# zakuro-ai/asr

Measured on AMD Instinct MI355X. Metric: utterances/sec (10 s, 161-bin) DS2 5x1024 BiGRU CTC train step, higher is better.
Workload: dtype bf16

## Files before the change

asr_amd/_lib.py:

```python
from __future__ import annotations

import ctypes as C
import os
from typing import Optional

_HERE = os.path.dirname(os.path.abspath(__file__))
LIB_PATH = os.environ.get("DS2_LIB_PATH") or os.path.join(_HERE, "lib", "libds2hip.so")

_lib: Optional[C.CDLL] = None

vp, i32, i64, f32, f64, sz = C.c_void_p, C.c_int, C.c_longlong, C.c_float, C.c_double, C.c_size_t

SIGNATURES = {
    "ds2_version": (C.c_char_p, []),
    "ds2_last_error": (C.c_char_p, []),
    "ds2_device_info": (i32, [C.POINTER(i32), C.POINTER(i32), C.c_char_p, i32]),
    "ds2_debug_flags": (i32, [vp, i32]),
    "ds2_rnn_ctx_init": (i32, [vp, vp, vp, vp]),
    "ds2_memset_async": (i32, [vp, i32, sz, vp]),
    "ds2_ablation_build": (i32, []),
    "ds2_rnn_persistent_status": (i32, [vp, vp]),
    "ds2_rnn_persistent_counters": (i32, [vp, vp]),
    "ds2_rnn_poison_if_starved": (i32, [vp, vp, sz, vp]),
    "ds2_rnn_poison_seen": (i32, [vp]),
# ... 21 lines not shown
    "ds2_cast_f32_from_bf16": (i32, [vp, vp, i64, vp]),
    "ds2_rnn_fwd_x": (i32, [vp, i32, vp, vp, vp, vp, vp, vp, vp, i32, i32, i32, vp, vp, vp, vp, sz, vp]),
    "ds2_split_bf16": (i32, [vp, i32, vp, i32, i32, i32, i32, vp]),
    "ds2_cast_transpose_bf16": (i32, [vp, i32, vp, i32, i32, i32, vp]),
    "ds2_cast_bf16_both_workspace_bytes": (sz, [i32, i32]),
    "ds2_cast_bf16_both": (i32, [vp, i32, vp, i32, vp, i32, i32, i32, vp, vp, sz, vp]),
    "ds2_transpose_bf16": (i32, [vp, i32, vp, i32, i32, i32, vp, vp, sz, vp]),
    "ds2_colreduce_workspace_bytes": (sz, [i32, i32]),
    "ds2_colstats_f32": (i32, [vp, i32, i32, i32, vp, vp, vp, vp, f32, vp, sz, vp]),
    "ds2_add_colstats_f32": (i32, [vp, i32, vp, i32, vp, i32, i32, i32, vp, vp, vp, vp, f32, vp, sz, vp]),
    "ds2_colsum_f32": (i32, [vp, i32, i32, i32, vp, vp, vp, sz, vp]),
    "ds2_bn1d_apply_f32": (i32, [vp, i32, vp, i32, i32, i32, vp, vp, vp, vp, f32, vp]),
    "ds2_bn1d_apply_bf16": (i32, [vp, i32, vp, i32, i32, i32, vp, vp, vp, vp, f32, vp]),
    "ds2_bn1d_bwd_f32": (i32, [vp, i32, vp, i32, vp, i32, i32, i32, vp, vp, vp, f32, vp, vp, vp, sz, vp]),
    "ds2_bn1d_bwd_xbf16": (i32, [vp, i32, vp, i32, vp, i32, i32, i32, vp, vp, vp, f32, vp, vp, vp, sz, vp]),
    "ds2_center_colstats": (i32, [vp, i32, vp, i32, vp, i32, vp, i32, i32, i32, vp, vp, vp, vp, vp, f32, vp, sz, vp]),
    "ds2_wih_fold_bf16": (i32, [vp, i32, vp, i32, i32, vp, vp, vp, vp, f32, vp, i32, vp, vp, vp, vp]),
    "ds2_scale_rank1_f32": (i32, [vp, i32, i32, i32, vp, vp, vp, vp]),
    "ds2_chanreduce_workspace_bytes": (sz, [i32]),
    "ds2_bn2d_stats_f32": (i32, [vp, i32, i32, i32, i32, vp, vp, vp, vp, f32, vp, sz, vp]),
    "ds2_bn2d_act_fwd_f32": (i32, [vp, vp, i32, i32, i32, i32, vp, vp, vp, vp, vp, f32, vp]),
    "ds2_bn2d_act_bwd_f32": (i32, [vp, vp, vp, i32, i32, i32, i32, vp, vp, vp, vp, vp, f32, vp, vp, vp, sz, vp]),
    "ds2_bn2d_act_fwd_fused": (i32, [vp, i32, i32, i32, vp, vp, vp, vp, vp, f32, vp, vp, vp, vp]),
    "ds2_bn2d_act_collapse": (i32, [vp, i32, i32, i32, vp, vp, vp, vp, vp, f32, vp, vp, i32, vp]),
    "ds2_bn2d_act_bwd_fused_workspace_bytes": (sz, [i32, i32, i32]),
    "ds2_bn2d_act_bwd_fused": (i32, [vp, vp, i32, i32, i32, vp, vp, vp, vp, vp, f32, vp, vp, vp, vp, vp, vp, vp, sz, vp]),
    "ds2_transpose_bft_f32": (i32, [vp, vp, i32, i32, i32, i32, vp]),
    "ds2_transpose2d_f32": (i32, [vp, i32, i64, vp, i32, i64, i32, i32, i32, vp]),
    "ds2_conv_dims": (None, [i32, i32, C.POINTER(i32), C.POINTER(i32), C.POINTER(i32)]),
    "ds2_conv_packed_floats": (sz, [i32]),
# ... 122 lines not shown
```

asr_amd/csrc/conv_bf16.hip:

```cpp
#include "common.h"
#include <stdlib.h>

namespace {

typedef __bf16 bf16x8 __attribute__((ext_vector_type(8)));

constexpr int TT = 128, KT = 11, PT = 5, CH = 32;
constexpr int NPIX = TT + KT - 1;
constexpr int IPITCH = 80;
constexpr int WROW = KT * 2 * 2 * 32 * 16;

__device__ __attribute__((aligned(16))) float g_zero_cb[4] = {0.f, 0.f, 0.f, 0.f};

struct CArgs {
  const __bf16* in;
  const __bf16* wpk;
  const float* bias;
  float* out;
  const int* lens;
  int B, Din, T, Dtot, KD, SD, PD, OS, OO;
  int gx, gy, gz;
};

constexpr int IN_CHUNKS = NPIX * 4;
// ... 18 lines not shown
    bx = pair % a.gx; bz = pair / a.gx;
  }
  const int t0 = bx * TT, o0 = R * by, b = bz;
  const int len = a.lens ? min(a.lens[b], a.T) : a.T;
  const int t = t0 + wave * 32 + l31;
  auto out_ptr = [&](int o, int co) { return a.out + (((long long)b * CH + co) * a.Dtot + (a.OS * o + a.OO)) * a.T + t; };
  if (t0 >= len) {
    if (t < a.T) {
#pragma unroll
      for (int q = 0; q < R; ++q)
        if (o0 + q < n_out) {
#pragma unroll
          for (int r = 0; r < 16; ++r) *out_ptr(o0 + q, (r & 3) + 8 * (r >> 2) + 4 * half) = 0.f;
        }
    }
    return;
  }
  f32x16 acc[R];
#pragma unroll
  for (int q = 0; q < R; ++q)
#pragma unroll
    for (int r = 0; r < 16; ++r) acc[q][r] = 0.f;

  const int f0 = SD * o0 - a.PD;
  f32x4 ri[IN_IT], rw[W_IT];
  auto load_in = [&](int f) {
    const bool rowok = f >= 0 && f < a.Din;
    const char* rowp = reinterpret_cast<const char*>(a.in + (((long long)b * a.Din + (rowok ? f : 0)) * a.T) * CH);
#pragma unroll
    for (int u = 0; u < IN_IT; ++u) {
// ... 166 lines not shown
  return 0;
}

extern "C" int ds2_conv2_fwd_bf16_stat_blocks(int B, int D1, int T) {
  const int D2 = (D1 + 2 * 10 - 21) / 2 + 1;
  return ceil_div(T, TT) * ceil_div(D2, 3) * B;
}

extern "C" int ds2_conv2_fwd_bf16_stats(const void* a1_nhwc, const void* wf, const float* bias, const int* lens_dev, float* y2, int B, int D1,
                                        int T, float* stat_part, void* stream) {
  DS2_REQUIRE(a1_nhwc && wf && y2, "ds2_conv2_fwd_bf16: null pointer");
  const int D2 = (D1 + 2 * 10 - 21) / 2 + 1;
  CArgs a{};
  a.in = (const __bf16*)a1_nhwc; a.wpk = (const __bf16*)wf; a.bias = bias; a.out = y2; a.lens = lens_dev;
  a.B = B; a.Din = D1; a.T = T; a.Dtot = D2; a.KD = 21; a.SD = 2; a.PD = 10; a.OS = 1; a.OO = 0;
  if (stat_part) DS2_HIP(hipMemsetAsync(stat_part, 0, (size_t)ds2_conv2_fwd_bf16_stat_blocks(B, D1, T) * 64 * sizeof(float), (hipStream_t)stream));
  a.gx = ceil_div(T, TT); a.gy = ceil_div(D2, 3); a.gz = B;
  hipLaunchKernelGGL((conv2_bf16_rows_kernel<2, 3>), dim3(a.gx * a.gy * a.gz), dim3(256), 0, (hipStream_t)stream, a, D2, stat_part);
  DS2_LAUNCH_CHECK("conv2_bf16_rows_kernel fwd");
  return 0;
}

extern "C" int ds2_conv2_fwd_bf16(const void* a1_nhwc, const void* wf, const float* bias, const int* lens_dev, float* y2, int B, int D1,
                                  int T, void* stream) {
  return ds2_conv2_fwd_bf16_stats(a1_nhwc, wf, bias, lens_dev, y2, B, D1, T, nullptr, stream);
}

extern "C" int ds2_conv2_dgrad_bf16(const void* dy2_nhwc, const void* wd0, const void* wd1, float* da1, int B, int D1, int T, void* stream) {
  DS2_REQUIRE(dy2_nhwc && wd0 && wd1 && da1, "ds2_conv2_dgrad_bf16: null pointer");
  const int D2 = (D1 + 2 * 10 - 21) / 2 + 1;
  for (int p = 0; p < 2; ++p) {
// ... 422 lines not shown
```

asr_amd/csrc/norm.hip:

```cpp
#include "common.h"
#include <algorithm>

namespace {

typedef float f32x4_dw __attribute__((ext_vector_type(4), aligned(4)));
typedef __bf16 nbf16x4 __attribute__((ext_vector_type(4)));
constexpr int BN_ROWS_PER_BLOCK = 32;
__device__ __forceinline__ f32x4 ld4(const float* __restrict__ p, int valid, bool vec) {
  f32x4 v = {0.f, 0.f, 0.f, 0.f};
  if (valid >= 4 && vec) {
    v = *reinterpret_cast<const f32x4*>(p);
  } else if (valid >= 4) {
    const f32x4_dw q = *reinterpret_cast<const f32x4_dw*>(p);
    v.x = q.x; v.y = q.y; v.z = q.z; v.w = q.w;
  } else {
    if (valid > 0) v.x = p[0];
    if (valid > 1) v.y = p[1];
    if (valid > 2) v.z = p[2];
    if (valid > 3) v.w = p[3];
  }
  return v;
}
__device__ __forceinline__ void st4(float* __restrict__ p, f32x4 v, int valid, bool vec) {
  if (valid >= 4 && vec) {
// ... 48 lines not shown
  red[rg][cq * 4 + 0][0] = s0.x; red[rg][cq * 4 + 0][1] = s1.x;
  red[rg][cq * 4 + 1][0] = s0.y; red[rg][cq * 4 + 1][1] = s1.y;
  red[rg][cq * 4 + 2][0] = s0.z; red[rg][cq * 4 + 2][1] = s1.z;
  red[rg][cq * 4 + 3][0] = s0.w; red[rg][cq * 4 + 3][1] = s1.w;
  __syncthreads();
  if (threadIdx.x < 128) {
    const int c = threadIdx.x >> 1, w = threadIdx.x & 1;
    float s = 0.f;
#pragma unroll
    for (int g = 0; g < 16; ++g) s += red[g][c][w];
    const int col = blockIdx.x * 64 + c;
    if (col < H) part[((long long)blockIdx.y * H + col) * 2 + w] = s;
  }
}

__global__ __launch_bounds__(256) void col_finalize_kernel(const float* __restrict__ part, int chunks, int H, double count, int kind,
                                                           float* __restrict__ out0, float* __restrict__ out1,
                                                           float* __restrict__ run_mean, float* __restrict__ run_var, float momentum) {
  __shared__ double red[8][32][2];
  const int cl = threadIdx.x & 31, grp = threadIdx.x >> 5;
  const int c = blockIdx.x * 32 + cl;
  double a = 0.0, b = 0.0;
  if (c < H) {
    double a1 = 0.0, b1 = 0.0, a2 = 0.0, b2 = 0.0, a3 = 0.0, b3 = 0.0;
    int k = grp;
    for (; k + 24 < chunks; k += 32) {
      const float2 p0 = *reinterpret_cast<const float2*>(part + ((long long)k * H + c) * 2);
      const float2 p1 = *reinterpret_cast<const float2*>(part + ((long long)(k + 8) * H + c) * 2);
      const float2 p2 = *reinterpret_cast<const float2*>(part + ((long long)(k + 16) * H + c) * 2);
      const float2 p3 = *reinterpret_cast<const float2*>(part + ((long long)(k + 24) * H + c) * 2);
      a += (double)p0.x; b += (double)p0.y; a1 += (double)p1.x; b1 += (double)p1.y;
      a2 += (double)p2.x; b2 += (double)p2.y; a3 += (double)p3.x; b3 += (double)p3.y;
    }
    for (; k < chunks; k += 8) {
      a += (double)part[((long long)k * H + c) * 2 + 0];
      b += (double)part[((long long)k * H + c) * 2 + 1];
// ... 14 lines not shown
  }
  if (kind == 0) {
    const double m = a / count;
    double v = b / count - m * m;
    if (v < 0.0) v = 0.0;
    out0[c] = (float)m;
    out1[c] = (float)v;
    if (run_mean) {
      const double unb = count > 1.0 ? v * count / (count - 1.0) : v;
      run_mean[c] = (float)((1.0 - momentum) * (double)run_mean[c] + momentum * m);
      run_var[c] = (float)((1.0 - momentum) * (double)run_var[c] + momentum * unb);
    }
  } else {
    out0[c] = (float)a;
    if (out1) out1[c] = (float)b;
  }
}

template <bool OUT_BF16>
__global__ __launch_bounds__(256) void bn1d_apply_kernel(const float* __restrict__ X, int ldx, void* __restrict__ Yv, int ldy, int M, int H,
                                                         const float* __restrict__ mean, const float* __restrict__ var,
                                                         const float* __restrict__ gamma, const float* __restrict__ beta, float eps, int vec) {
  const int c0 = (blockIdx.x * 256 + threadIdx.x) * 4;
  const int wcols = OUT_BF16 ? ldy : H;
  if (c0 >= wcols) return;
  const int valid = H - c0;
  f32x4 sc = {0.f, 0.f, 0.f, 0.f}, sh = {0.f, 0.f, 0.f, 0.f};
  if (valid > 0) {
    const f32x4 mu = ld4(mean + c0, valid, false), vv = ld4(var + c0, valid, false);
    const f32x4 g = ld4(gamma + c0, valid, false), b = ld4(beta + c0, valid, false);
// ... 578 lines not shown
  int vec = (ldx % 4 == 0) && ((uintptr_t)X % 16 == 0);
  if (X2) vec = vec && (ldx2 % 4 == 0) && ((uintptr_t)X2 % 16 == 0);
  if (Y) vec = vec && (ldy % 4 == 0) && ((uintptr_t)Y % 16 == 0);
  dim3 grid(colblocks, nch), block(256);
  float* part = (float*)ws;
  if (mode == 0) hipLaunchKernelGGL((col_reduce_kernel<0>), grid, block, 0, s, X, ldx, X2, ldx2, Y, ldy, M, H, rpc, mean, var, eps, part, vec);
  else if (mode == 1) hipLaunchKernelGGL((col_reduce_kernel<1>), grid, block, 0, s, X, ldx, X2, ldx2, Y, ldy, M, H, rpc, mean, var, eps, part, vec);
  else hipLaunchKernelGGL((col_reduce_kernel<2>), grid, block, 0, s, X, ldx, X2, ldx2, Y, ldy, M, H, rpc, mean, var, eps, part, vec);
  DS2_LAUNCH_CHECK("col_reduce_kernel");
  hipLaunchKernelGGL(col_finalize_kernel, dim3(ceil_div(H, 32)), dim3(256), 0, s, (const float*)part, nch, H, (double)M, kind,
                     out0, out1, run_mean, run_var, momentum);
  DS2_LAUNCH_CHECK("col_finalize_kernel");
  return 0;
}

int ds2i_col_finalize_sums(const float* part, int chunks, int H, float* out0, float* out1, hipStream_t s) {
  hipLaunchKernelGGL(col_finalize_kernel, dim3(ceil_div(H, 32)), dim3(256), 0, s, part, chunks, H, 1.0, 1, out0, out1, (float*)nullptr,
                     (float*)nullptr, 0.f);
  DS2_LAUNCH_CHECK("col_finalize_kernel");
  return 0;
}

extern "C" int ds2_colstats_f32(const float* X, int ldx, int M, int H, float* mean, float* var, float* run_mean, float* run_var,
                                float momentum, void* ws, size_t ws_bytes, void* stream) {
  DS2_REQUIRE(X && mean && var && M > 0 && H > 0, "ds2_colstats_f32: bad args");
  return col_reduce_launch(0, X, ldx, nullptr, 0, nullptr, 0, M, H, nullptr, nullptr, 0.f, 0, mean, var, run_mean, run_var,
                           momentum, ws, ws_bytes, (hipStream_t)stream);
}

extern "C" int ds2_add_colstats_f32(const float* Xa, int lda, const float* Xb, int ldb, float* Y, int ldy, int M, int H,
// ... 95 lines not shown
  const int colblocks = ceil_div(H, 64);
  const int chunks = pick_chunks(M, colblocks, 64);
  const int rpc = ceil_div(M, chunks);
  const int nch = ceil_div(M, rpc);
  DS2_REQUIRE(ws && ws_bytes >= (size_t)nch * H * 2 * sizeof(float), "ds2_bn1d_bwd_xbf16: workspace too small");
  const int vec = (lddy % 4 == 0) && ((uintptr_t)dY % 16 == 0);
  hipStream_t s = (hipStream_t)stream;
  hipLaunchKernelGGL(col_reduce_bwd_xbf_kernel, dim3(colblocks, nch), dim3(256), 0, s, (const __bf16*)X_bf16, ldx, dY, lddy, M, H, rpc, mean, var, eps,
                     (float*)ws, vec);
  DS2_LAUNCH_CHECK("col_reduce_bwd_xbf_kernel");
  hipLaunchKernelGGL(col_finalize_kernel, dim3(ceil_div(H, 32)), dim3(256), 0, s, (const float*)ws, nch, H, (double)M, 1, dbeta, dgamma, (float*)nullptr,
                     (float*)nullptr, 0.f);
  DS2_LAUNCH_CHECK("col_finalize_kernel");
  if (!dX) return 0;
  return ds2i_bn1d_bwd_apply_xbf(dY, lddy, X_bf16, ldx, dX, lddx, M, H, mean, var, gamma, dbeta, dgamma, eps, s);
}

extern "C" int ds2_scale_rank1_f32(float* C, int ldc, int R, int N, const float* scale, const float* rowv, const float* shift, void* stream) {
  DS2_REQUIRE(C && scale && rowv && shift && R > 0 && N > 0 && (N % 4) == 0 && (ldc % 4) == 0 && ((uintptr_t)C % 16) == 0 &&
              ((uintptr_t)scale % 16) == 0 && ((uintptr_t)shift % 16) == 0, "ds2_scale_rank1_f32: bad args");
  const long long total = (long long)R * (N / 4);
  const int blocks = (int)std::min<long long>((total + 255) / 256, 8192);
  hipLaunchKernelGGL(scale_rank1_kernel, dim3(blocks), dim3(256), 0, (hipStream_t)stream, C, ldc, R, N, scale, rowv, shift);
  DS2_LAUNCH_CHECK("scale_rank1_kernel");
  return 0;
}

extern "C" size_t ds2_chanreduce_workspace_bytes(int C) { return (size_t)2048 * 2 * sizeof(float) * (size_t)(C > 1 ? C : 1); }

static int chan_reduce_launch(int mode, const float* Y, const float* dA, int Bn, int C, int D, int T, const int* lens,
// ... 187 lines not shown
```

asr_amd/engine.py:

```python
from __future__ import annotations

from dataclasses import dataclass, field
from typing import Dict, List, Optional

import torch

from . import _lib, ops

Tensor = torch.Tensor
import os as _os
def _tune(name: str, default: str) -> str:
    return _os.environ.get(name, default) if _os.environ.get("DS2_EXPERIMENTAL") == "1" else default


OVERLAP_MODE = _tune("DS2_OVERLAP", "2")
OVERLAP_WGRAD = OVERLAP_MODE == "1"
WGRAD_TN = _tune("DS2_WGRAD_TN", "1") != "0"
CONV_STATS = _tune("DS2_CONV_STATS", "1") != "0"
FUSE_BN_BWD = _tune("DS2_FUSE_BN_BWD", "1") != "0"
WGRAD_SIDE = _tune("DS2_WGRAD_SIDE", "sk")
WGRAD_IDLE = _tune("DS2_WGRAD_IDLE", "1") != "0"
WGRAD_IDLE_MIN_CUS = int(_tune("DS2_WGRAD_IDLE_MIN_CUS", "64"))
F32_GEMM = _os.environ.get("DS2_F32_GEMM", "split")

# ... 33 lines not shown
    if key not in _SIDE:
        _SIDE[key] = torch.cuda.Stream(device=device)
    return _SIDE[key]


@dataclass
class BnGrad:
    dyn: Tensor
    x: Tensor
    mean: Tensor
    var: Tensor
    gamma: Tensor
    sums: tuple


def _bn_backward(dxn: Tensor, x: Tensor, mean, var, gamma, dgamma, dbeta, fuse: bool, private_sums: bool):
    xbf = x.dtype == torch.bfloat16
    if not fuse:
        return (ops.bn1d_bwd_xbf if xbf else ops.bn1d_bwd)(dxn, x, mean, var, gamma, dgamma, dbeta)
    sums_fn = ops.bn1d_bwd_sums_xbf if xbf else ops.bn1d_bwd_sums
    if private_sums:
        sums = sums_fn(dxn, x, mean, var, gamma)
        dbeta.copy_(sums[0])
        dgamma.copy_(sums[1])
    else:
        sums = sums_fn(dxn, x, mean, var, gamma, out=(dbeta, dgamma))
    return BnGrad(dxn, x, mean, var, gamma, sums)


@dataclass
class ModelCfg:
    rnn: str
    hidden: int
    layers: int
    classes: int
# ... 127 lines not shown
    else:
        a2 = ops.bn2d_act_fwd(y2, lens_dev, m2, v2, W[cp + "4.weight"], W[cp + "4.bias"])
        xin = ops.transpose_bft(a2, B, 32 * D2, T, to_tbf=True).view(M, 32 * D2)
        del a2
    if save:
        ctx.y1, ctx.a1, ctx.a1p, ctx.y2, ctx.st1, ctx.st2 = y1, a1, a1p, y2, (m1, v1), (m2, v2)

    mean = var = delta = None
    bf = cfg.precision == "bf16"
    prep = None
    if bf and save:
        may_fold = (BN_FOLD and training and B % 8 == 0 and H % 8 == 0 and OVERLAP_MODE == "2" and T > 1
                    and (BN_FOLD_IDLE or not _wgrad_idle_schedule(x.device, B, H)))
        prep = ops.weight_prep_bf16([(G, W[f"rnns.{l}.whh_cat"], W[f"rnns.{l}.wih_cat"],
                                      xn0.shape[1] if l == 0 else (None if may_fold else ops._pad8(H))) for l in range(L)])
    for l in range(L):
        lc = LayerCtx()
        rmode = 1 if bf else (2 if (F32_RNN == "split" and H % 32 == 0) else 0)
        ws_f = ops.rnn_ws("fwd", G, B, H, rmode, x.device) if WS_PREARM else None
        folded = l > 0 and xin.dtype == torch.bfloat16
        if folded:
            bp = f"rnns.{l}.batch_norm.module."
            xn = xin
            w_bf, bias_eff, colscale, colshift = ops.wih_fold(W[f"rnns.{l}.wih_cat"], W[f"rnns.{l}.bih_cat"], var, W[bp + "weight"], W[bp + "bias"], delta,
                                                              ld=xn.shape[1])
            lc.wihT = prep[l][2] if prep is not None else ops.cast_transpose_bf16(W[f"rnns.{l}.wih_cat"])
            lc.mean, lc.var, lc.fold = delta, var, (colscale, colshift)
            gx = ops.gemm_bf16_nt(xn, w_bf, bias=bias_eff)
            del w_bf
        elif l > 0:
            bp = f"rnns.{l}.batch_norm.module."
            if not training:
                mean, var = W[bp + "running_mean"], W[bp + "running_var"]
            xn = (ops.bn1d_apply_bf16 if cfg.precision == "bf16" else ops.bn1d_apply)(xin, mean, var, W[bp + "weight"], W[bp + "bias"])
# ... 35 lines not shown
                        and (BN_FOLD_IDLE or not _wgrad_idle_schedule(x.device, B, H))) else None)
            hbuf, aux, rec = ops.rnn_fwd(G, gx, wpf, W[f"rnns.{l}.bhh_cat"], lens_dev, T, B, H, bf16=True, packed_gates=True, h_bf16=h_bf, ws=ws_f, hsum=hsum)
            if hsum is not None and not (ops.rnn_last_path(x.device) & 1):
                hsum = None
            gx = None
            lc.rec, lc.gshape = rec, (M, 2 * G * H)
            if h_bf is not None and (ops.rnn_last_path(x.device) & 1):
                lc.h_bf = h_bf
        else:
            hsum = None
            hbuf, aux = ops.rnn_fwd(G, gx, wpf, W[f"rnns.{l}.bhh_cat"], lens_dev, T, B, H, bf16=rmode, ws=ws_f)
        lc.wpb = wpb
        nxt = f"rnns.{l + 1}.batch_norm.module" if l + 1 < L else "fc.0.module.0"
        if hsum is not None:
            y, mean, var, delta = ops.center_colstats(hbuf[:, :H], hbuf[:, H:], hsum, *run(nxt))
        else:
            y, mean, var = ops.add_colstats(hbuf[:, :H], hbuf[:, H:], *run(nxt))
        if save:
            lc.xin, lc.xn, lc.gx, lc.hbuf, lc.aux = xin, xn, gx, hbuf, aux
            ctx.layers.append(lc)
        xin = y

    fp = "fc.0.module."
    if not training:
        mean, var = W[fp + "0.running_mean"], W[fp + "0.running_var"]
    xn = ops.bn1d_apply(xin, mean, var, W[fp + "0.weight"], W[fp + "0.bias"])
    logits = ops.gemm(xn, W[fp + "1.weight"], transB=True)
    if save:
        ctx.y_last, ctx.fc_xn, ctx.fc_stats = xin, xn, (mean, var)
    if training:
        if "_bn_counters" in W:
            ops.add_i64(W["_bn_counters"], 1)
        else:
            for name in ([cp + "1", cp + "4", fp + "0"] + [f"rnns.{l}.batch_norm.module" for l in range(1, L)]):
                W[name + ".num_batches_tracked"] += 1
    return logits.view(T, B, cfg.classes), ctx


def _backward_rnn_deferred(W, Gr, cfg: ModelCfg, ctx: Ctx, dy, done, private: bool, serial_buckets: bool = False):
    G, H, L = cfg.gates, cfg.hidden, cfg.layers
    B, T = ctx.B, ctx.T
    M = T * B
    lens_dev = ctx.lens_dev
    main = torch.cuda.current_stream()
    dev = ctx.lens_dev.device
    side = _side_stream(dev)
    pending = None
    report = done

    def done(name):
        if name == "rnns.0" and getattr(ctx, "side_used", False) and not serial_buckets:
            torch.cuda.current_stream().wait_stream(side)
        report(name)

# ... 95 lines not shown
            for t in (dgx_bf, aux, hbuf, xn):
                if t is not None:
                    t.record_stream(side)
        return (l, dgxT, hT, auxT, xnT, ready, (dgx_bf,))

    queued = None
    queued_tn = None
    queued_side = None
    queued_idle = None
    group_ok = WGRAD_SIDE != "0" and W[f"rnns.0.wih_cat"].shape[1] % 8 == 0
    side_ok = group_ok and WGRAD_SIDE == "1" and ops.wgrad_fits_beside_bwd_recurrence(G, H)
    n_idle = _idle_cus_beside_bwd_recurrence(dev, B, H)
    idle_ok = (group_ok and WGRAD_SIDE == "sk" and WGRAD_IDLE and T > 1
               and WGRAD_IDLE_MIN_CUS <= n_idle < torch.cuda.get_device_properties(dev).multi_processor_count // 2)
    fold_of = {l: ctx.layers[l].fold for l in range(L)}
    ws_b = ops.rnn_ws("bwd", G, B, H, 1, dev) if WS_PREARM else None
    for l in range(L - 1, -1, -1):
        lc = ctx.layers[l]
        if queued_side is not None:
            start = torch.cuda.Event()
            start.record(main)
            weight_gradients_group(*queued_side, True, start)
            queued_side = None
        if queued is not None:
            start = torch.cuda.Event()
            start.record(main)
            pending = operand_passes(*queued, start)
            queued = None
        start_idle = None
        if queued_idle is not None:
            start_idle = torch.cuda.Event()
# ... 9 lines not shown
            ops.rnn_bwd(G, dy, lc.gx, lc.aux, lc.hbuf, lc.wpb, lens_dev, T, B, H, bf16=True, dgx_bf16=dgx_bf, gates_bf16=lc.rec, dhn_bf16=dhn_bf,
                        bias_part=bias_part, ws=ws_b)
        _BWD_PERSISTENT[shape_key] = bool(ops.rnn_last_path(dev) & 2)
        if queued_idle is not None:
            weight_gradients_group(*queued_idle, _BWD_PERSISTENT[shape_key], start_idle)
            queued_idle = None
        tn = want_tn and _BWD_PERSISTENT[shape_key]
        lc.rec = None
        if pending is not None:
            weight_gradients(pending)
            pending = None
        if tn:
            queued_tn = (l, dgx_bf, dhn_bf, lc.h_bf, lc.xn, bias_part)
        else:
            queued = (l, (lc.aux, lc.hbuf, lc.xn), dgx_bf)
        ws_b = ops.rnn_ws("bwd", G, B, H, 1, dev) if (WS_PREARM and l > 0) else None
        dxn = ops.gemm_bf16_nt(dgx_bf, (lc.wihT if lc.wihT is not None else ops.cast_transpose_bf16(W[f"rnns.{l}.wih_cat"])))
        if l > 0:
            bp = f"rnns.{l}.batch_norm.module."
            dy = _bn_backward(dxn, lc.xin, lc.mean, lc.var, W[bp + "weight"], Gr[bp + "weight"], Gr[bp + "bias"], FUSE_BN_BWD, private)
        else:
            dy = dxn
        del dxn
        if tn and group_ok:
            ops.rnn_bias_grads(G, bias_part, Gr[f"rnns.{l}.bih_cat"], Gr[f"rnns.{l}.bhh_cat"])
            if side_ok:
                queued_side = queued_tn[:5]
            elif idle_ok and l > 0:
                queued_idle = queued_tn[:5]
            else:
                weight_gradients_group(*queued_tn[:5], False, None)
            queued_tn = None
        elif tn:
            weight_gradients_tn(*queued_tn)
            queued_tn = None
        lc.gx = lc.aux = lc.hbuf = lc.xn = lc.wpb = lc.h_bf = lc.wihT = None
    if queued_side is not None:
        start = torch.cuda.Event()
        start.record(main)
        weight_gradients_group(*queued_side, True, start)
# ... 11 lines not shown
    main = torch.cuda.current_stream()
    f32_key = (ops.rnn_ctx_key(dlogits.device), G, H, ctx.B, "f32")
    idle_f32 = (cfg.precision != "bf16" and WGRAD_IDLE and _BWD_PERSISTENT.get(f32_key, False)
                and _idle_cus_beside_bwd_recurrence(dlogits.device, ctx.B, H) >= WGRAD_IDLE_MIN_CUS)
    side = _side_stream(dlogits.device) if (OVERLAP_WGRAD or idle_f32) else main
    keep = []
    B, T, D1, D2 = ctx.B, ctx.T, ctx.D1, ctx.D2
    M = T * B
    lens_dev = ctx.lens_dev
    dl = dlogits.reshape(M, Cn)
    fp = "fc.0.module."
    ops.gemm(dl, ctx.fc_xn, transA=True, out=Gr[fp + "1.weight"])
    dxn = ops.gemm(dl, W[fp + "1.weight"])
    mean, var = ctx.fc_stats
    deferred = OVERLAP_MODE == "2" and cfg.precision == "bf16" and B % 8 == 0 and T > 1
    dy = _bn_backward(dxn, ctx.y_last, mean, var, W[fp + "0.weight"], Gr[fp + "0.weight"], Gr[fp + "0.bias"], FUSE_BN_BWD and deferred,
                      on_bucket is not None)
    del dxn
    done("fc")
    if deferred:
        serial = getattr(getattr(on_bucket, "__self__", None), "mode", None) == "serial"
        dy = _backward_rnn_deferred(W, Gr, cfg, ctx, dy, done, on_bucket is not None, serial)
        first_layer = -1
    else:
        first_layer = L - 1
    defer = idle_f32 and not OVERLAP_WGRAD
    pending_off = None
    for l in range(first_layer, -1, -1):
        lc = ctx.layers[l]
        bf = cfg.precision == "bf16"
        split = (not bf) and lc.xs is not None
        bfd = bf and B % 8 == 0
        gshape = lc.gx.shape if lc.gx is not None else lc.gshape
        dgx_bf = torch.empty(gshape, dtype=torch.bfloat16, device=dy.device) if bfd else None
        rmode = 1 if bf else (2 if (F32_RNN == "split" and H % 32 == 0) else 0)
        ops.rnn_bwd(G, dy, lc.gx, lc.aux, lc.hbuf, lc.wpb, lens_dev, T, B, H, bf16=rmode, dgx_bf16=dgx_bf, gates_bf16=lc.rec)
        if not bf:
# ... 200 lines not shown
```

asr_amd/ops.py:

```python
from __future__ import annotations

import ctypes as C
import threading
from typing import Optional, Tuple

import torch

from . import _lib

Tensor = torch.Tensor
BN_EPS = 1e-5
BN_MOMENTUM = 0.1


def _ptr(t: Optional[Tensor]):
    return None if t is None else t.data_ptr()


def _stream():
    return torch.cuda.current_stream().cuda_stream


def _chk_f32(*ts):
    for t in ts:
# ... 393 lines not shown


def colstats(X: Tensor, run_mean: Optional[Tensor] = None, run_var: Optional[Tensor] = None):
    _chk_f32(X, run_mean, run_var)
    lib = _lib.load()
    M, H = X.shape
    mean = torch.empty(H, dtype=torch.float32, device=X.device)
    var = torch.empty_like(mean)
    wsb = lib.ds2_colreduce_workspace_bytes(M, H)
    ws = _ws(wsb, X.device)
    _lib.check(lib.ds2_colstats_f32(X.data_ptr(), _row_pitch(X), M, H, mean.data_ptr(), var.data_ptr(), _ptr(run_mean),
                                    _ptr(run_var), BN_MOMENTUM, ws.data_ptr(), wsb, _stream()), "ds2_colstats_f32")
    return mean, var


def add_colstats(Xa: Tensor, Xb: Tensor, run_mean: Optional[Tensor] = None, run_var: Optional[Tensor] = None):
    _chk_f32(Xa, Xb, run_mean, run_var)
    lib = _lib.load()
    M, H = Xa.shape
    Y = torch.empty(M, H, dtype=torch.float32, device=Xa.device)
    mean = torch.empty(H, dtype=torch.float32, device=Xa.device)
    var = torch.empty_like(mean)
    wsb = lib.ds2_colreduce_workspace_bytes(M, H)
    ws = _ws(wsb, Xa.device)
    _lib.check(lib.ds2_add_colstats_f32(Xa.data_ptr(), _row_pitch(Xa), Xb.data_ptr(), _row_pitch(Xb), Y.data_ptr(), H, M, H,
                                        mean.data_ptr(), var.data_ptr(), _ptr(run_mean), _ptr(run_var), BN_MOMENTUM,
                                        ws.data_ptr(), wsb, _stream()), "ds2_add_colstats_f32")
    return Y, mean, var


def center_colstats(Xa: Tensor, Xb: Tensor, hsum: Tensor, run_mean: Optional[Tensor] = None, run_var: Optional[Tensor] = None):
    _chk_f32(Xa, Xb, hsum, run_mean, run_var)
# ... 445 lines not shown
                wr = torch.empty(R, ld_r, dtype=torch.bfloat16, device=wih.device)
                e.wih_r, e.ld_r = wr.data_ptr(), ld_r
        out.append((wpf, wpb, wt, wr))
    _lib.check(lib.ds2_weight_prep_bf16(tab, len(layers), _stream()), "ds2_weight_prep_bf16")
    return out


def rnn_ws(kind: str, gates: int, B: int, H: int, bf16, device) -> Tensor:
    lib = _lib.load()
    n = lib.ds2_rnn_fwd_workspace_bytes(B, H, int(bf16)) if kind == "fwd" else lib.ds2_rnn_bwd_workspace_bytes(gates, B, H, int(bf16))
    ws = _ws(n, device)
    _lib.check(lib.ds2_memset_async(ws.data_ptr(), 0xff, ws.numel(), _stream()), "ds2_memset_async")
    return ws


def _take_ws(ws: Optional[Tensor], need: int, device):
    if ws is None:
        return _ws(need, device), False
    assert ws.numel() >= need and ws.device == torch.device(device)
    return ws, True


def _rnn_call(device, armed: bool, thunk):
    ctx = rnn_ctx(device)
    ctx.ws_prearmed = 1 if armed else 0
    try:
        return thunk()
    finally:
        ctx.ws_prearmed = 0

# ... 105 lines not shown

def bn1d_bwd_sums(dY: Tensor, X: Tensor, mean: Tensor, var: Tensor, gamma: Tensor, out: Optional[Tuple[Tensor, Tensor]] = None) -> Tuple[Tensor, Tensor]:
    _chk_f32(dY, X, mean, var, gamma)
    lib = _lib.load()
    M, H = X.shape
    if out is None:
        both = torch.empty(2, H, dtype=torch.float32, device=X.device)
        out = (both[0], both[1])
    s0, s1 = out
    _chk_f32(s0, s1)
    assert s0.is_contiguous() and s1.is_contiguous() and s0.numel() == H == s1.numel()
    wsb = lib.ds2_colreduce_workspace_bytes(M, H)
    ws = _ws(wsb, X.device)
    _lib.check(lib.ds2_bn1d_bwd_f32(dY.data_ptr(), _row_pitch(dY), X.data_ptr(), _row_pitch(X), None, 0, M, H, mean.data_ptr(), var.data_ptr(),
                                    gamma.data_ptr(), BN_EPS, s1.data_ptr(), s0.data_ptr(), ws.data_ptr(), wsb, _stream()), "ds2_bn1d_bwd_f32")
    return s0, s1


def rnn_bwd_bn(gates: int, dyn: Tensor, bn_x: Tensor, mean: Tensor, var: Tensor, gamma: Tensor, sums: Tensor, gx: Optional[Tensor], aux: Optional[Tensor],
               hbuf: Tensor, wp_bwd: Tensor, lens_dev: Tensor, T: int, B: int, H: int, bf16: bool = False, dgx_bf16: Optional[Tensor] = None,
               gates_bf16: Optional[Tensor] = None, dhn_bf16: Optional[Tensor] = None, bias_part: Optional[Tensor] = None, ws: Optional[Tensor] = None):
    s0, s1 = sums
    xbf = bn_x.dtype == torch.bfloat16
    _chk_f32(dyn, None if xbf else bn_x, mean, var, gamma, s0, s1, gx, aux, hbuf, bias_part)
    assert s0.is_contiguous() and s1.is_contiguous() and s0.numel() == H == s1.numel() and bn_x.shape[0] == T * B and bn_x.shape[1] >= H and dyn.shape == (T * B, H)
    assert bn_x.stride(1) == 1 and (not xbf or bn_x.shape[1] == H or bn_x.stride(0) % 2 == 0)
    lib = _lib.load()
    wsb = lib.ds2_rnn_bwd_workspace_bytes(gates, B, H, int(bf16))
    ws, armed = _take_ws(ws, wsb, dyn.device)
    def call(scratch):
# ... 370 lines not shown
```

include/ds2hip.h:

```cpp
#ifndef DS2HIP_H
#define DS2HIP_H

#include <stddef.h>
#include <stdint.h>

#ifdef __cplusplus
extern "C" {
#endif

const char* ds2_version(void);
const char* ds2_last_error(void);
int ds2_device_info(int* cu_count, int* wave_size, char* arch, int arch_len);
int ds2_ablation_build(void);

typedef struct ds2_rnn_ctx {
  int size;
  int persist_fwd, persist_bwd;
  int cooldown;
  int rearm_calls;
  int starved_total;
  int last_path;
  int last_bwd_kind;
  int debug_flags;
  int ws_prearmed;
// ... 49 lines not shown
int ds2_bn1d_apply_bf16(const float* X, int ldx, void* Y, int ldy, int M, int H, const float* mean, const float* var, const float* gamma,
                        const float* beta, float eps, void* stream);
int ds2_bn1d_bwd_f32(const float* dY, int lddy, const float* X, int ldx, float* dX, int lddx, int M, int H, const float* mean,
                     const float* var, const float* gamma, float eps, float* dgamma, float* dbeta, void* ws, size_t ws_bytes,
                     void* stream);

int ds2_center_colstats(const float* Xa, int lda, const float* Xb, int ldb, const float* hsum, int ntiles, void* Yc_bf16, int ldyc, int M, int H,
                        float* mean, float* var, float* delta, float* run_mean, float* run_var, float momentum, void* ws, size_t ws_bytes,
                        void* stream);
int ds2_wih_fold_bf16(const float* W, int ldw, const float* bias, int R, int I, const float* var, const float* gamma, const float* beta,
                      const float* delta, float eps, void* W2_bf16, int ldw2, float* bias2, float* colscale, float* colshift, void* stream);
int ds2_scale_rank1_f32(float* C, int ldc, int R, int N, const float* scale, const float* rowv, const float* shift, void* stream);
int ds2_bn1d_bwd_xbf16(const float* dY, int lddy, const void* X_bf16, int ldx, float* dX, int lddx, int M, int H, const float* mean, const float* var,
                       const float* gamma, float eps, float* dgamma, float* dbeta, void* ws, size_t ws_bytes, void* stream);

size_t ds2_chanreduce_workspace_bytes(int C);
int ds2_bn2d_stats_f32(const float* Y, int B, int C, int D, int T, float* mean, float* var, float* run_mean, float* run_var,
                       float momentum, void* ws, size_t ws_bytes, void* stream);
int ds2_bn2d_act_fwd_f32(const float* Y, float* A, int B, int C, int D, int T, const int* lens_dev, const float* mean,
                         const float* var, const float* gamma, const float* beta, float eps, void* stream);
int ds2_bn2d_act_bwd_f32(const float* Y, const float* dA, float* dY, int B, int C, int D, int T, const int* lens_dev, const float* mean,
                         const float* var, const float* gamma, const float* beta, float eps, float* dgamma, float* dbeta, void* ws,
                         size_t ws_bytes, void* stream);

int ds2_bn2d_act_fwd_fused(const float* Y, int B, int D, int T, const int* lens_dev, const float* mean, const float* var,
                           const float* gamma, const float* beta, float eps, float* a_f32, void* a_pad, void* a_nhwc, void* stream);
int ds2_bn2d_act_collapse(const float* Y, int B, int D, int T, const int* lens_dev, const float* mean, const float* var,
                          const float* gamma, const float* beta, float eps, float* x_f32, void* x_bf16, int ld_bf, void* stream);
size_t ds2_bn2d_act_bwd_fused_workspace_bytes(int B, int D, int T);
int ds2_bn2d_act_bwd_fused(const float* Y, const float* dA, int B, int D, int T, const int* lens_dev, const float* mean,
// ... 176 lines not shown
```

Before: 2861.

## Fold small tail launches into grouped finalize kernels and batch RNN workspace arming

Adds a grouped finalize kernel that, besides the BN column-stat finalize, also reduces RNN bias gradients, bumps the BN step counters, and fills RNN workspace memory. This takes several tiny kernel and memset launches off the critical stream. RNN forward and backward workspaces are now allocated and armed once per pass as one block instead of per layer. The conv2 stats memset is replaced by zeroing inside early-exit blocks. The cost is more complex coupling between unrelated jobs and more places where correctness depends on every block zeroing or writing its slot.

```diff
diff --git a/asr_amd/_lib.py b/asr_amd/_lib.py
--- a/asr_amd/_lib.py
+++ b/asr_amd/_lib.py
@@ -59,6 +59,8 @@
     "ds2_bn1d_apply_bf16": (i32, [vp, i32, vp, i32, i32, i32, vp, vp, vp, vp, f32, vp]),
     "ds2_bn1d_bwd_f32": (i32, [vp, i32, vp, i32, vp, i32, i32, i32, vp, vp, vp, f32, vp, vp, vp, sz, vp]),
     "ds2_bn1d_bwd_xbf16": (i32, [vp, i32, vp, i32, vp, i32, i32, i32, vp, vp, vp, f32, vp, vp, vp, sz, vp]),
+    "ds2_add_colstats_cnt_f32": (i32, [vp, i32, vp, i32, vp, i32, i32, i32, vp, vp, vp, vp, f32, vp, i32, i64, vp, sz, vp]),
+    "ds2_bn1d_bwd_sums_group": (i32, [vp, i32, vp, i32, i32, i32, i32, vp, vp, f32, vp, vp, i32, vp, i32, i32, vp, vp, vp, sz, i32, vp, sz, vp]),
     "ds2_center_colstats": (i32, [vp, i32, vp, i32, vp, i32, vp, i32, i32, i32, vp, vp, vp, vp, vp, f32, vp, sz, vp]),
     "ds2_wih_fold_bf16": (i32, [vp, i32, vp, i32, i32, vp, vp, vp, vp, f32, vp, i32, vp, vp, vp, vp]),
     "ds2_scale_rank1_f32": (i32, [vp, i32, i32, i32, vp, vp, vp, vp]),
diff --git a/asr_amd/csrc/conv_bf16.hip b/asr_amd/csrc/conv_bf16.hip
--- a/asr_amd/csrc/conv_bf16.hip
+++ b/asr_amd/csrc/conv_bf16.hip
@@ -56,6 +56,7 @@
           for (int r = 0; r < 16; ++r) *out_ptr(o0 + q, (r & 3) + 8 * (r >> 2) + 4 * half) = 0.f;
         }
     }
+    if (stat_part && tid < 64) stat_part[((((long long)bz * a.gy + by) * a.gx + bx) * 32 + (tid >> 1)) * 2 + (tid & 1)] = 0.f;
     return;
   }
   f32x16 acc[R];
@@ -252,7 +253,6 @@
   CArgs a{};
   a.in = (const __bf16*)a1_nhwc; a.wpk = (const __bf16*)wf; a.bias = bias; a.out = y2; a.lens = lens_dev;
   a.B = B; a.Din = D1; a.T = T; a.Dtot = D2; a.KD = 21; a.SD = 2; a.PD = 10; a.OS = 1; a.OO = 0;
-  if (stat_part) DS2_HIP(hipMemsetAsync(stat_part, 0, (size_t)ds2_conv2_fwd_bf16_stat_blocks(B, D1, T) * 64 * sizeof(float), (hipStream_t)stream));
   a.gx = ceil_div(T, TT); a.gy = ceil_div(D2, 3); a.gz = B;
   hipLaunchKernelGGL((conv2_bf16_rows_kernel<2, 3>), dim3(a.gx * a.gy * a.gz), dim3(256), 0, (hipStream_t)stream, a, D2, stat_part);
   DS2_LAUNCH_CHECK("conv2_bf16_rows_kernel fwd");
diff --git a/asr_amd/csrc/norm.hip b/asr_amd/csrc/norm.hip
--- a/asr_amd/csrc/norm.hip
+++ b/asr_amd/csrc/norm.hip
@@ -86,12 +86,12 @@
   }
 }
 
-__global__ __launch_bounds__(256) void col_finalize_kernel(const float* __restrict__ part, int chunks, int H, double count, int kind,
-                                                           float* __restrict__ out0, float* __restrict__ out1,
-                                                           float* __restrict__ run_mean, float* __restrict__ run_var, float momentum) {
+__device__ __forceinline__ void col_finalize_block(int bx, const float* __restrict__ part, int chunks, int H, double count, int kind,
+                                                   float* __restrict__ out0, float* __restrict__ out1,
+                                                   float* __restrict__ run_mean, float* __restrict__ run_var, float momentum) {
   __shared__ double red[8][32][2];
   const int cl = threadIdx.x & 31, grp = threadIdx.x >> 5;
-  const int c = blockIdx.x * 32 + cl;
+  const int c = bx * 32 + cl;
   double a = 0.0, b = 0.0;
   if (c < H) {
     double a1 = 0.0, b1 = 0.0, a2 = 0.0, b2 = 0.0, a3 = 0.0, b3 = 0.0;
@@ -136,6 +136,63 @@
   } else {
     out0[c] = (float)a;
     if (out1) out1[c] = (float)b;
+  }
+}
+__global__ __launch_bounds__(256) void col_finalize_kernel(const float* __restrict__ part, int chunks, int H, double count, int kind,
+                                                           float* __restrict__ out0, float* __restrict__ out1,
+                                                           float* __restrict__ run_mean, float* __restrict__ run_var, float momentum) {
+  col_finalize_block(blockIdx.x, part, chunks, H, count, kind, out0, out1, run_mean, run_var, momentum);
+}
+
+struct FinGroup {
+  const float* part; int chunks, H; double count; int kind; float* out0; float* out1; float* run_mean; float* run_var; float momentum;
+  int ncf;
+  const float* bias_part; int B, Hb, G; float* dbih; float* dbhh; int nbias;
+  long long* cnt; int ncnt; long long add;
+  uint4* fill; long long fill16; unsigned pattern; int nfill;
+};
+__global__ __launch_bounds__(256) void finalize_group_kernel(FinGroup g) {
+  int bx = blockIdx.x;
+  if (bx < g.ncf) {
+    col_finalize_block(bx, g.part, g.chunks, g.H, g.count, g.kind, g.out0, g.out1, g.run_mean, g.run_var, g.momentum);
+    return;
+  }
+  bx -= g.ncf;
+  if (bx < g.nbias) {
+    const int H = g.Hb, G = g.G, B = g.B;
+    const int idx = bx * 256 + threadIdx.x;
+    if (idx >= 2 * 4 * H) return;
+    const int j = idx % H, slot = (idx / H) & 3, dir = idx / (4 * H);
+    if (G == 1 && slot != 0) return;
+    const float* __restrict__ part = g.bias_part;
+    float s = 0.f;
+    int b = 0;
+    for (; b + 8 <= B; b += 8) {
+      float v[8];
+#pragma unroll
+      for (int k = 0; k < 8; ++k) v[k] = part[(long long)(b + k) * 8 * H + idx];
+#pragma unroll
+      for (int k = 0; k < 8; ++k) s += v[k];
+    }
+    for (; b < B; ++b) s += part[(long long)b * 8 * H + idx];
+    const long long o = (long long)dir * G * H + j;
+    if (G == 4 || G == 1) { g.dbih[o + slot * H] = s; g.dbhh[o + slot * H] = s; }
+    else if (slot < 2) { g.dbih[o + slot * H] = s; g.dbhh[o + slot * H] = s; }
+    else if (slot == 2) g.dbih[o + 2 * H] = s;
+    else g.dbhh[o + 2 * H] = s;
+    return;
+  }
+  bx -= g.nbias;
+  if (g.ncnt > 0) {
+    if (bx == 0) {
+      for (int i = threadIdx.x; i < g.ncnt; i += 256) g.cnt[i] += g.add;
+      return;
+    }
+    bx -= 1;
+  }
+  if (bx < g.nfill) {
+    const uint4 v = {g.pattern, g.pattern, g.pattern, g.pattern};
+    for (long long i = (long long)bx * 256 + threadIdx.x; i < g.fill16; i += (long long)g.nfill * 256) g.fill[i] = v;
   }
 }
 
@@ -744,6 +801,19 @@
   return 0;
 }
 
+static int finalize_group_launch(FinGroup g, const float* part, int chunks, int H, double count, int kind, float* out0, float* out1, float* run_mean,
+                                 float* run_var, float momentum, hipStream_t s) {
+  g.part = part; g.chunks = chunks; g.H = H; g.count = count; g.kind = kind; g.out0 = out0; g.out1 = out1; g.run_mean = run_mean; g.run_var = run_var;
+  g.momentum = momentum;
+  g.ncf = ceil_div(H, 32);
+  g.nbias = g.bias_part ? ceil_div(8 * g.Hb, 256) : 0;
+  g.nfill = g.fill16 > 0 ? (int)std::min<long long>((g.fill16 + 2047) / 2048, 512) : 0;
+  const int blocks = g.ncf + g.nbias + (g.ncnt > 0 ? 1 : 0) + g.nfill;
+  hipLaunchKernelGGL(finalize_group_kernel, dim3(blocks), dim3(256), 0, s, g);
+  DS2_LAUNCH_CHECK("finalize_group_kernel");
+  return 0;
+}
+
 int ds2i_col_finalize_sums(const float* part, int chunks, int H, float* out0, float* out1, hipStream_t s) {
   hipLaunchKernelGGL(col_finalize_kernel, dim3(ceil_div(H, 32)), dim3(256), 0, s, part, chunks, H, 1.0, 1, out0, out1, (float*)nullptr,
                      (float*)nullptr, 0.f);
@@ -869,6 +939,59 @@
   DS2_LAUNCH_CHECK("col_finalize_kernel");
   if (!dX) return 0;
   return ds2i_bn1d_bwd_apply_xbf(dY, lddy, X_bf16, ldx, dX, lddx, M, H, mean, var, gamma, dbeta, dgamma, eps, s);
+}
+
+extern "C" int ds2_add_colstats_cnt_f32(const float* Xa, int lda, const float* Xb, int ldb, float* Y, int ldy, int M, int H, float* mean, float* var,
+                                        float* run_mean, float* run_var, float momentum, long long* cnt, int ncnt, long long add, void* ws,
+                                        size_t ws_bytes, void* stream) {
+  DS2_REQUIRE(Xa && Xb && Y && mean && var && M > 0 && H > 0 && ncnt >= 0, "ds2_add_colstats_cnt_f32: bad args");
+  const int colblocks = ceil_div(H, 64);
+  const int chunks = pick_chunks(M, colblocks, 64);
+  const int rpc = ceil_div(M, chunks);
+  const int nch = ceil_div(M, rpc);
+  DS2_REQUIRE(ws && ws_bytes >= (size_t)nch * H * 2 * sizeof(float), "ds2_add_colstats_cnt_f32: workspace too small");
+  const int vec = (lda % 4 == 0) && ((uintptr_t)Xa % 16 == 0) && (ldb % 4 == 0) && ((uintptr_t)Xb % 16 == 0) && (ldy % 4 == 0) && ((uintptr_t)Y % 16 == 0);
+  hipStream_t s = (hipStream_t)stream;
+  float* part = (float*)ws;
+  hipLaunchKernelGGL((col_reduce_kernel<1>), dim3(colblocks, nch), dim3(256), 0, s, Xa, lda, Xb, ldb, Y, ldy, M, H, rpc, (const float*)nullptr,
+                     (const float*)nullptr, 0.f, part, vec);
+  DS2_LAUNCH_CHECK("col_reduce_kernel");
+  FinGroup g{};
+  if (cnt && ncnt > 0) { g.cnt = cnt; g.ncnt = ncnt; g.add = add; }
+  return finalize_group_launch(g, part, nch, H, (double)M, 0, mean, var, run_mean, run_var, momentum, s);
+}
+
+extern "C" int ds2_bn1d_bwd_sums_group(const float* dY, int lddy, const void* X, int ldx, int x_bf16, int M, int H, const float* mean, const float* var,
+                                       float eps, float* dgamma, float* dbeta, int gates, const float* bias_part, int Bb, int Hb, float* dbih,
+                                       float* dbhh, void* fill, size_t fill_bytes, int fill_value, void* ws, size_t ws_bytes, void* stream) {
+  DS2_REQUIRE(dY && X && mean && var && dgamma && dbeta && M > 0 && H > 0, "ds2_bn1d_bwd_sums_group: bad args");
+  DS2_REQUIRE(!x_bf16 || (ldx % 4) == 0, "ds2_bn1d_bwd_sums_group: the bf16 operand's pitch must be a multiple of 4");
+  DS2_REQUIRE(!bias_part || ((gates == 1 || gates == 3 || gates == 4) && dbih && dbhh && Bb > 0 && Hb > 0), "ds2_bn1d_bwd_sums_group: bad bias job");
+  DS2_REQUIRE(!fill || ((fill_bytes % 16) == 0 && ((uintptr_t)fill % 16) == 0), "ds2_bn1d_bwd_sums_group: the fill must be whole 16-byte chunks");
+  const int colblocks = ceil_div(H, 64);
+  const int chunks = pick_chunks(M, colblocks, 64);
+  const int rpc = ceil_div(M, chunks);
+  const int nch = ceil_div(M, rpc);
+  DS2_REQUIRE(ws && ws_bytes >= (size_t)nch * H * 2 * sizeof(float), "ds2_bn1d_bwd_sums_group: workspace too small");
+  hipStream_t s = (hipStream_t)stream;
+  float* part = (float*)ws;
+  if (x_bf16) {
+    const int vec = (lddy % 4 == 0) && ((uintptr_t)dY % 16 == 0);
+    hipLaunchKernelGGL(col_reduce_bwd_xbf_kernel, dim3(colblocks, nch), dim3(256), 0, s, (const __bf16*)X, ldx, dY, lddy, M, H, rpc, mean, var, eps, part, vec);
+    DS2_LAUNCH_CHECK("col_reduce_bwd_xbf_kernel");
+  } else {
+    const int vec = (ldx % 4 == 0) && ((uintptr_t)X % 16 == 0) && (lddy % 4 == 0) && ((uintptr_t)dY % 16 == 0);
+    hipLaunchKernelGGL((col_reduce_kernel<2>), dim3(colblocks, nch), dim3(256), 0, s, (const float*)X, ldx, dY, lddy, (float*)nullptr, 0, M, H, rpc, mean,
+                       var, eps, part, vec);
+    DS2_LAUNCH_CHECK("col_reduce_kernel");
+  }
+  FinGroup g{};
+  if (bias_part) { g.bias_part = bias_part; g.B = Bb; g.Hb = Hb; g.G = gates; g.dbih = dbih; g.dbhh = dbhh; }
+  if (fill && fill_bytes) {
+    const unsigned b = (unsigned)fill_value & 0xffu;
+    g.fill = (uint4*)fill; g.fill16 = (long long)(fill_bytes / 16); g.pattern = b * 0x01010101u;
+  }
+  return finalize_group_launch(g, part, nch, H, (double)M, 1, dbeta, dgamma, nullptr, nullptr, 0.f, s);
 }
 
 extern "C" int ds2_scale_rank1_f32(float* C, int ldc, int R, int N, const float* scale, const float* rowv, const float* shift, void* stream) {
diff --git a/asr_amd/engine.py b/asr_amd/engine.py
--- a/asr_amd/engine.py
+++ b/asr_amd/engine.py
@@ -71,11 +71,16 @@
     sums: tuple
 
 
-def _bn_backward(dxn: Tensor, x: Tensor, mean, var, gamma, dgamma, dbeta, fuse: bool, private_sums: bool):
+def _bn_backward(dxn: Tensor, x: Tensor, mean, var, gamma, dgamma, dbeta, fuse: bool, private_sums: bool, bias=None, fill=None):
     xbf = x.dtype == torch.bfloat16
     if not fuse:
+        assert bias is None and fill is None
         return (ops.bn1d_bwd_xbf if xbf else ops.bn1d_bwd)(dxn, x, mean, var, gamma, dgamma, dbeta)
-    sums_fn = ops.bn1d_bwd_sums_xbf if xbf else ops.bn1d_bwd_sums
+    if bias is not None or fill is not None:
+        def sums_fn(*a, **kw):
+            return ops.bn1d_bwd_sums_group(*a, bias=bias, fill=fill, **kw)
+    else:
+        sums_fn = ops.bn1d_bwd_sums_xbf if xbf else ops.bn1d_bwd_sums
     if private_sums:
         sums = sums_fn(dxn, x, mean, var, gamma)
         dbeta.copy_(sums[0])
@@ -233,10 +238,12 @@
                     and (BN_FOLD_IDLE or not _wgrad_idle_schedule(x.device, B, H)))
         prep = ops.weight_prep_bf16([(G, W[f"rnns.{l}.whh_cat"], W[f"rnns.{l}.wih_cat"],
                                       xn0.shape[1] if l == 0 else (None if may_fold else ops._pad8(H))) for l in range(L)])
+    rmode = 1 if bf else (2 if (F32_RNN == "split" and H % 32 == 0) else 0)
+    ws_f_all = ops.rnn_ws_many("fwd", L, G, B, H, rmode, x.device)[1] if WS_PREARM else None
+    counted = False
     for l in range(L):
         lc = LayerCtx()
-        rmode = 1 if bf else (2 if (F32_RNN == "split" and H % 32 == 0) else 0)
-        ws_f = ops.rnn_ws("fwd", G, B, H, rmode, x.device) if WS_PREARM else None
+        ws_f = ws_f_all[l] if WS_PREARM else None
         folded = l > 0 and xin.dtype == torch.bfloat16
         if folded:
             bp = f"rnns.{l}.batch_norm.module."
@@ -302,6 +309,9 @@
         nxt = f"rnns.{l + 1}.batch_norm.module" if l + 1 < L else "fc.0.module.0"
         if hsum is not None:
             y, mean, var, delta = ops.center_colstats(hbuf[:, :H], hbuf[:, H:], hsum, *run(nxt))
+        elif bf and training and l == L - 1 and "_bn_counters" in W:
+            y, mean, var = ops.add_colstats(hbuf[:, :H], hbuf[:, H:], *run(nxt), counters=W["_bn_counters"])
+            counted = True
         else:
             y, mean, var = ops.add_colstats(hbuf[:, :H], hbuf[:, H:], *run(nxt))
         if save:
@@ -316,7 +326,7 @@
     logits = ops.gemm(xn, W[fp + "1.weight"], transB=True)
     if save:
         ctx.y_last, ctx.fc_xn, ctx.fc_stats = xin, xn, (mean, var)
-    if training:
+    if training and not counted:
         if "_bn_counters" in W:
             ops.add_i64(W["_bn_counters"], 1)
         else:
@@ -325,7 +335,7 @@
     return logits.view(T, B, cfg.classes), ctx
 
 
-def _backward_rnn_deferred(W, Gr, cfg: ModelCfg, ctx: Ctx, dy, done, private: bool, serial_buckets: bool = False):
+def _backward_rnn_deferred(W, Gr, cfg: ModelCfg, ctx: Ctx, dy, done, private: bool, serial_buckets: bool = False, ws_all=None):
     G, H, L = cfg.gates, cfg.hidden, cfg.layers
     B, T = ctx.B, ctx.T
     M = T * B
@@ -451,7 +461,9 @@
     idle_ok = (group_ok and WGRAD_SIDE == "sk" and WGRAD_IDLE and T > 1
                and WGRAD_IDLE_MIN_CUS <= n_idle < torch.cuda.get_device_properties(dev).multi_processor_count // 2)
     fold_of = {l: ctx.layers[l].fold for l in range(L)}
-    ws_b = ops.rnn_ws("bwd", G, B, H, 1, dev) if WS_PREARM else None
+    if WS_PREARM and ws_all is None:
+        ws_all = ops.rnn_ws_many("bwd", L, G, B, H, 1, dev)[1]
+    ws_b = ws_all[L - 1] if WS_PREARM else None
     for l in range(L - 1, -1, -1):
         lc = ctx.layers[l]
         if queued_side is not None:
@@ -491,16 +503,18 @@
             queued_tn = (l, dgx_bf, dhn_bf, lc.h_bf, lc.xn, bias_part)
         else:
             queued = (l, (lc.aux, lc.hbuf, lc.xn), dgx_bf)
-        ws_b = ops.rnn_ws("bwd", G, B, H, 1, dev) if (WS_PREARM and l > 0) else None
+        ws_b = ws_all[l - 1] if (WS_PREARM and l > 0) else None
         dxn = ops.gemm_bf16_nt(dgx_bf, (lc.wihT if lc.wihT is not None else ops.cast_transpose_bf16(W[f"rnns.{l}.wih_cat"])))
+        bias_job = (G, bias_part, Gr[f"rnns.{l}.bih_cat"], Gr[f"rnns.{l}.bhh_cat"]) if (tn and group_ok and l > 0 and FUSE_BN_BWD) else None
         if l > 0:
             bp = f"rnns.{l}.batch_norm.module."
-            dy = _bn_backward(dxn, lc.xin, lc.mean, lc.var, W[bp + "weight"], Gr[bp + "weight"], Gr[bp + "bias"], FUSE_BN_BWD, private)
+            dy = _bn_backward(dxn, lc.xin, lc.mean, lc.var, W[bp + "weight"], Gr[bp + "weight"], Gr[bp + "bias"], FUSE_BN_BWD, private, bias=bias_job)
         else:
             dy = dxn
         del dxn
         if tn and group_ok:
-            ops.rnn_bias_grads(G, bias_part, Gr[f"rnns.{l}.bih_cat"], Gr[f"rnns.{l}.bhh_cat"])
+            if bias_job is None:
+                ops.rnn_bias_grads(G, bias_part, Gr[f"rnns.{l}.bih_cat"], Gr[f"rnns.{l}.bhh_cat"])
             if side_ok:
                 queued_side = queued_tn[:5]
             elif idle_ok and l > 0:
@@ -542,13 +556,16 @@
     dxn = ops.gemm(dl, W[fp + "1.weight"])
     mean, var = ctx.fc_stats
     deferred = OVERLAP_MODE == "2" and cfg.precision == "bf16" and B % 8 == 0 and T > 1
+    ws_whole, ws_all = (ops.rnn_ws_many("bwd", L, G, B, H, 1, dlogits.device, arm=False)
+                        if (deferred and FUSE_BN_BWD and WS_PREARM) else (None, None))
     dy = _bn_backward(dxn, ctx.y_last, mean, var, W[fp + "0.weight"], Gr[fp + "0.weight"], Gr[fp + "0.bias"], FUSE_BN_BWD and deferred,
-                      on_bucket is not None)
+                      on_bucket is not None, fill=ws_whole)
+    del ws_whole
     del dxn
     done("fc")
     if deferred:
         serial = getattr(getattr(on_bucket, "__self__", None), "mode", None) == "serial"
-        dy = _backward_rnn_deferred(W, Gr, cfg, ctx, dy, done, on_bucket is not None, serial)
+        dy = _backward_rnn_deferred(W, Gr, cfg, ctx, dy, done, on_bucket is not None, serial, ws_all)
         first_layer = -1
     else:
         first_layer = L - 1
diff --git a/asr_amd/ops.py b/asr_amd/ops.py
--- a/asr_amd/ops.py
+++ b/asr_amd/ops.py
@@ -431,8 +431,21 @@
     return mean, var
 
 
-def add_colstats(Xa: Tensor, Xb: Tensor, run_mean: Optional[Tensor] = None, run_var: Optional[Tensor] = None):
+def add_colstats(Xa: Tensor, Xb: Tensor, run_mean: Optional[Tensor] = None, run_var: Optional[Tensor] = None, counters: Optional[Tensor] = None):
     _chk_f32(Xa, Xb, run_mean, run_var)
+    if counters is not None:
+        assert counters.dtype == torch.int64 and counters.is_contiguous() and counters.is_cuda
+        lib = _lib.load()
+        M, H = Xa.shape
+        Y = torch.empty(M, H, dtype=torch.float32, device=Xa.device)
+        mean = torch.empty(H, dtype=torch.float32, device=Xa.device)
+        var = torch.empty_like(mean)
+        wsb = lib.ds2_colreduce_workspace_bytes(M, H)
+        ws = _ws(wsb, Xa.device)
+        _lib.check(lib.ds2_add_colstats_cnt_f32(Xa.data_ptr(), _row_pitch(Xa), Xb.data_ptr(), _row_pitch(Xb), Y.data_ptr(), H, M, H,
+                                                mean.data_ptr(), var.data_ptr(), _ptr(run_mean), _ptr(run_var), BN_MOMENTUM,
+                                                counters.data_ptr(), counters.numel(), 1, ws.data_ptr(), wsb, _stream()), "ds2_add_colstats_cnt_f32")
+        return Y, mean, var
     lib = _lib.load()
     M, H = Xa.shape
     Y = torch.empty(M, H, dtype=torch.float32, device=Xa.device)
@@ -908,6 +921,16 @@
     return ws
 
 
+def rnn_ws_many(kind: str, n: int, gates: int, B: int, H: int, bf16, device, arm: bool = True):
+    lib = _lib.load()
+    need = lib.ds2_rnn_fwd_workspace_bytes(B, H, int(bf16)) if kind == "fwd" else lib.ds2_rnn_bwd_workspace_bytes(gates, B, H, int(bf16))
+    pitch = (max(int(need), 16) + 255) // 256 * 256
+    whole = torch.empty(n * pitch, dtype=torch.uint8, device=device)
+    if arm:
+        _lib.check(lib.ds2_memset_async(whole.data_ptr(), 0xff, whole.numel(), _stream()), "ds2_memset_async")
+    return whole, [whole[i * pitch:(i + 1) * pitch] for i in range(n)]
+
+
 def _take_ws(ws: Optional[Tensor], need: int, device):
     if ws is None:
         return _ws(need, device), False
@@ -1043,6 +1066,38 @@
     ws = _ws(wsb, X.device)
     _lib.check(lib.ds2_bn1d_bwd_f32(dY.data_ptr(), _row_pitch(dY), X.data_ptr(), _row_pitch(X), None, 0, M, H, mean.data_ptr(), var.data_ptr(),
                                     gamma.data_ptr(), BN_EPS, s1.data_ptr(), s0.data_ptr(), ws.data_ptr(), wsb, _stream()), "ds2_bn1d_bwd_f32")
+    return s0, s1
+
+
+def bn1d_bwd_sums_group(dY: Tensor, X: Tensor, mean: Tensor, var: Tensor, gamma: Tensor, out: Optional[Tuple[Tensor, Tensor]] = None,
+                        bias: Optional[tuple] = None, fill: Optional[Tensor] = None, fill_value: int = 0xff) -> Tuple[Tensor, Tensor]:
+    _chk_f32(dY, mean, var, gamma)
+    xbf = X.dtype == torch.bfloat16
+    if not xbf:
+        _chk_f32(X)
+    assert X.is_cuda and X.stride(1) == 1
+    lib = _lib.load()
+    M, H = dY.shape
+    if out is None:
+        both = torch.empty(2, H, dtype=torch.float32, device=dY.device)
+        out = (both[0], both[1])
+    s0, s1 = out
+    _chk_f32(s0, s1)
+    assert s0.is_contiguous() and s1.is_contiguous() and s0.numel() == H == s1.numel()
+    g, bp, bb, hb, dbih, dbhh = 0, None, 0, 0, None, None
+    if bias is not None:
+        g, bp, dbih, dbhh = bias
+        _chk_f32(bp, dbih, dbhh)
+        bb, _, _, hb = bp.shape
+        assert bp.is_contiguous() and dbih.is_contiguous() and dbhh.is_contiguous() and dbih.numel() == 2 * g * hb == dbhh.numel()
+    if fill is not None:
+        assert fill.dtype == torch.uint8 and fill.is_contiguous() and fill.numel() % 16 == 0 and fill.data_ptr() % 16 == 0
+    wsb = lib.ds2_colreduce_workspace_bytes(M, H)
+    ws = _ws(wsb, dY.device)
+    _lib.check(lib.ds2_bn1d_bwd_sums_group(dY.data_ptr(), _row_pitch(dY), X.data_ptr(), X.stride(0), int(xbf), M, H, mean.data_ptr(), var.data_ptr(), BN_EPS,
+                                           s1.data_ptr(), s0.data_ptr(), int(g), _ptr(bp), int(bb), int(hb), _ptr(dbih), _ptr(dbhh), _ptr(fill),
+                                           fill.numel() if fill is not None else 0, int(fill_value), ws.data_ptr(), wsb, _stream()),
+               "ds2_bn1d_bwd_sums_group")
     return s0, s1
 
 
diff --git a/include/ds2hip.h b/include/ds2hip.h
--- a/include/ds2hip.h
+++ b/include/ds2hip.h
@@ -87,6 +87,13 @@
 int ds2_bn1d_bwd_xbf16(const float* dY, int lddy, const void* X_bf16, int ldx, float* dX, int lddx, int M, int H, const float* mean, const float* var,
                        const float* gamma, float eps, float* dgamma, float* dbeta, void* ws, size_t ws_bytes, void* stream);
 
+int ds2_add_colstats_cnt_f32(const float* Xa, int lda, const float* Xb, int ldb, float* Y, int ldy, int M, int H, float* mean, float* var,
+                             float* run_mean, float* run_var, float momentum, long long* cnt, int ncnt, long long add, void* ws, size_t ws_bytes,
+                             void* stream);
+int ds2_bn1d_bwd_sums_group(const float* dY, int lddy, const void* X, int ldx, int x_bf16, int M, int H, const float* mean, const float* var, float eps,
+                            float* dgamma, float* dbeta, int gates, const float* bias_part, int Bb, int Hb, float* dbih, float* dbhh, void* fill,
+                            size_t fill_bytes, int fill_value, void* ws, size_t ws_bytes, void* stream);
+
 size_t ds2_chanreduce_workspace_bytes(int C);
 int ds2_bn2d_stats_f32(const float* Y, int B, int C, int D, int T, float* mean, float* var, float* run_mean, float* run_var,
                        float momentum, void* ws, size_t ws_bytes, void* stream);
```

Result: no change. 2864, median of 5 (+0.1%).
